# Bissmella/Small-object-detection-transformers

Hardware: AMD Instinct MI355X
Metric: images/sec (1024x1024 RGB+IR) train fwd+bwd (higher is better)
Workload: dtype bf16; 1 GPU; SRyolo_MF.yaml (model.yaml graph), batch 8/GPU @ 1024x1024 RGB+IR, fwd + hand-written bwd + fused SGD-nesterov/weight-decay + EMA step, loss = YOLOv5 ComputeLoss (CIoU + BCE, device kernels), 32 synthetic boxes/image, random-init weights; global_batch=8, parallelism=dp1

## Files before the change

### small-object-detection-transformers_amd/csrc/convmlp.hip

```cpp
#include "common.h"
#include "launch.h"
#include "../../include/sodt_hip.h"

namespace {

constexpr int CT = 64, CK = 16;
constexpr int CONVMLP_MAXC = 384;
template <typename LA, typename LB>
__device__ __forceinline__ void tile64(float (&acc)[4][4], int K, float (*As)[CT + 1], float (*Bs)[CT + 1], LA la, LB lb, bool a_k_fast, bool b_k_fast) {
  const int tid = threadIdx.x, ty = tid >> 4, tx = tid & 15;
  float pa[4], pb[4];
  auto fetch = [&](int k0) {
#pragma unroll
    for (int e = 0; e < 4; ++e) {
      const int idx = tid + 256 * e;
      pa[e] = a_k_fast ? la(idx >> 4, k0 + (idx & 15)) : la(idx & 63, k0 + (idx >> 6));
      pb[e] = b_k_fast ? lb(k0 + (idx & 15), idx >> 4) : lb(k0 + (idx >> 6), idx & 63);
    }
  };
  fetch(0);
  for (int k0 = 0; k0 < K; k0 += CK) {
#pragma unroll
    for (int e = 0; e < 4; ++e) {
      const int idx = tid + 256 * e;
      if (a_k_fast) As[idx & 15][idx >> 4] = pa[e]; else As[idx >> 6][idx & 63] = pa[e];
      if (b_k_fast) Bs[idx & 15][idx >> 4] = pb[e]; else Bs[idx >> 6][idx & 63] = pb[e];
    }
    __syncthreads();
    if (k0 + CK < K) fetch(k0 + CK);
#pragma unroll
    for (int k = 0; k < CK; ++k) {
      float a[4], b[4];
#pragma unroll
      for (int i = 0; i < 4; ++i) { a[i] = As[k][ty + 16 * i]; b[i] = Bs[k][tx + 16 * i]; }
#pragma unroll
      for (int i = 0; i < 4; ++i)
#pragma unroll
        for (int j = 0; j < 4; ++j) acc[i][j] = fmaf(a[i], b[j], acc[i][j]);
    }
    __syncthreads();
  }
}

__global__ __launch_bounds__(256) void convmlp_compose_kernel(const float* __restrict__ W1, const float* __restrict__ b1,
                                                              const float* __restrict__ Wc, const float* __restrict__ bc,
                                                              bf16* __restrict__ weff, bf16* __restrict__ weffT,
                                                              float* __restrict__ beff, float* __restrict__ vtap, int C) {
  __shared__ float As[CT][CT + 1], Bs[CK][CT + 1];
  const int tid = threadIdx.x, t = blockIdx.z;
  if ((int)blockIdx.y == C / CT) {
    if (t != 0 || (int)blockIdx.x * 32 >= C) return;
    const int co = blockIdx.x * 32 + (tid >> 3), part = tid & 7;
    float a[4] = {0.f, 0.f, 0.f, 0.f};
    for (int m = part; m < C; m += 8) {
      const float4 w = *(const float4*)(Wc + ((long)co * C + m) * 4);
      const float b = b1[m];
      a[0] = fmaf(w.x, b, a[0]); a[1] = fmaf(w.y, b, a[1]); a[2] = fmaf(w.z, b, a[2]); a[3] = fmaf(w.w, b, a[3]);
    }
#pragma unroll
    for (int j = 0; j < 4; ++j) { a[j] += __shfl_xor(a[j], 1); a[j] += __shfl_xor(a[j], 2); a[j] += __shfl_xor(a[j], 4); }
    if (part == 0) {
#pragma unroll
      for (int j = 0; j < 4; ++j) vtap[j * C + co] = a[j];
      beff[co] = bc[co] + a[0] + a[1] + a[2] + a[3];
    }
    return;
  }
  if ((int)blockIdx.x >= C / CT) return;
  const int ci0 = blockIdx.x * CT, co0 = blockIdx.y * CT;
  float acc[4][4] = {};
  tile64(acc, C, (float (*)[CT + 1])As, Bs,
         [&](int r, int k) { return Wc[((long)(co0 + r) * C + k) * 4 + t]; },
         [&](int k, int c) { return W1[(long)k * C + ci0 + c]; }, true, false);
  const int ty = tid >> 4, tx = tid & 15;
#pragma unroll
  for (int i = 0; i < 4; ++i)
#pragma unroll
    for (int j = 0; j < 4; ++j) {
      weff[(long)(co0 + ty + 16 * i) * 4 * C + t * C + ci0 + tx + 16 * j] = (bf16)acc[i][j];
      As[tx + 16 * j][ty + 16 * i] = acc[i][j];
    }
  __syncthreads();
  for (int idx = tid; idx < CT * CT; idx += 256) {
    const int r = idx >> 6, c = idx & 63;
    weffT[(long)(ci0 + r) * 4 * C + t * C + co0 + c] = (bf16)As[r][c];
  }
}

__global__ __launch_bounds__(256) void convmlp_border_fix_kernel(bf16* __restrict__ cp, bf16* __restrict__ ca, const float* __restrict__ vtap,
                                                                 int B, int H, int W, int C) {
  const int nb = H + W - 1, cpr = C / 8;
  const long i = (long)blockIdx.x * 256 + threadIdx.x;
  if (i >= (long)B * nb * cpr) return;
  const int c8 = (int)(i % cpr) * 8;
  const int k = (int)((i / cpr) % nb), b = (int)(i / ((long)cpr * nb));
  const int y = k < W ? H - 1 : k - W, x = k < W ? k : W - 1;
  const bool bot = y == H - 1, rgt = x == W - 1;
  const long row = ((long)b * H + y) * W + x;
  float v[8];
  unpack<bf16>(*(const uint4*)(cp + row * C + c8), v);
#pragma unroll
  for (int j = 0; j < 8; ++j) {
    float s = 0.f;
    if (rgt) s += vtap[1 * C + c8 + j];
    if (bot) s += vtap[2 * C + c8 + j];
    if (rgt || bot) s += vtap[3 * C + c8 + j];
    v[j] -= s;
  }
  *(uint4*)(cp + row * C + c8) = pack<bf16>(v);
#pragma unroll
  for (int j = 0; j < 8; ++j) v[j] = gelu_t<bf16>(v[j]);
  *(uint4*)(ca + row * C + c8) = pack<bf16>(v);
}

__global__ __launch_bounds__(256) void convmlp_border_sums_kernel(const bf16* __restrict__ dc, float* __restrict__ bs, int B, int H, int W, int C) {
  __shared__ float red[8][392];
  const int b = blockIdx.y, kind = blockIdx.z;
  const int len = kind == 0 ? H : W;
  const int t = blockIdx.x * 8 + (threadIdx.x >> 5);
  const int cpr = C / 8;
  const bool ok = t < len;
  const int y = kind == 0 ? t : H - 1, x = kind == 0 ? W - 1 : t;
  for (int ch = threadIdx.x & 31; ch < cpr; ch += 32) {
    float v[8] = {0.f, 0.f, 0.f, 0.f, 0.f, 0.f, 0.f, 0.f};
    if (ok) unpack<bf16>(*(const uint4*)(dc + (((long)b * H + y) * W + x) * C + ch * 8), v);
#pragma unroll
    for (int j = 0; j < 8; ++j) red[threadIdx.x >> 5][ch * 8 + j] = v[j];
    if (ok && kind == 0 && t == H - 1)
#pragma unroll
      for (int j = 0; j < 8; ++j) atomicAdd(bs + 2 * C + ch * 8 + j, v[j]);
  }
  __syncthreads();
  for (int c = threadIdx.x; c < C; c += 256) {
    float a = 0.f;
#pragma unroll
    for (int r = 0; r < 8; ++r) a += red[r][c];
    atomicAdd(bs + kind * C + c, a);
  }
}

__global__ __launch_bounds__(256) void convmlp_decompose_kernel(const float* __restrict__ dweff, const float* __restrict__ colsum,
                                                                const float* __restrict__ bs, const float* __restrict__ W1,
                                                                const float* __restrict__ b1, const float* __restrict__ Wc,
                                                                float* __restrict__ gWc, float* __restrict__ gbc, float* __restrict__ gW1,
                                                                float* __restrict__ gb1, int C) {
  __shared__ float As[CK][CT + 1], Bs[CK][CT + 1];
  __shared__ float dvs[4 * CONVMLP_MAXC];
  const int tid = threadIdx.x, ty = tid >> 4, tx = tid & 15;
  const int nt = C / CT, n = nt * nt;
  auto dv = [&](int t, int co) {
    const float r = bs[co], bt = bs[C + co], cn = bs[2 * C + co];
    return colsum[co] - (t == 0 ? 0.f : t == 1 ? r : t == 2 ? bt : r + bt - cn);
  };
  int bid = blockIdx.x;
  if (bid < 4 * n) {
    const int t = bid & 3, tl = bid >> 2;
    const int m0 = (tl % nt) * CT, co0 = (tl / nt) * CT;
    float acc[4][4] = {};
    tile64(acc, C, As, Bs,
           [&](int r, int k) { return dweff[(long)(co0 + r) * 4 * C + t * C + k]; },
           [&](int k, int c) { return W1[(long)(m0 + c) * C + k]; }, true, true);
#pragma unroll
    for (int i = 0; i < 4; ++i)
#pragma unroll
      for (int j = 0; j < 4; ++j)
        gWc[((long)(co0 + ty + 16 * i) * C + m0 + tx + 16 * j) * 4 + t] += acc[i][j] + dv(t, co0 + ty + 16 * i) * b1[m0 + tx + 16 * j];
    return;
  }
  bid -= 4 * n;
  if (bid < 4 * n) {
    const int q = bid & 3, tl = bid >> 2;
    const int ci0 = (tl % nt) * CT, m0 = (tl / nt) * CT;
    const int kq = q * C;
    float acc[4][4] = {};
    tile64(acc, C, As, Bs,
           [&](int r, int k) { const int kk = kq + k; return Wc[((long)(kk >> 2) * C + m0 + r) * 4 + (kk & 3)]; },
           [&](int k, int c) { const int kk = kq + k; return dweff[(long)(kk >> 2) * 4 * C + (kk & 3) * C + ci0 + c]; }, true, false);
#pragma unroll
    for (int i = 0; i < 4; ++i)
#pragma unroll
      for (int j = 0; j < 4; ++j) atomicAdd(gW1 + (long)(m0 + ty + 16 * i) * C + ci0 + tx + 16 * j, acc[i][j]);
    return;
  }
  bid -= 4 * n;
  for (int i = tid; i < 4 * C; i += 256) dvs[i] = dv(i / C, i % C);
  __syncthreads();
  const int m = bid * 32 + (tid >> 3), part = tid & 7;
  float acc = 0.f;
  for (int co = part; co < C; co += 8) {
    const float4 wc = *(const float4*)(Wc + ((long)co * C + m) * 4);
    acc += wc.x * dvs[co] + wc.y * dvs[C + co] + wc.z * dvs[2 * C + co] + wc.w * dvs[3 * C + co];
  }
  acc += __shfl_xor(acc, 1); acc += __shfl_xor(acc, 2); acc += __shfl_xor(acc, 4);
  if (part == 0) {
    gb1[m] += acc;
    gbc[m] += colsum[m];
  }
}

inline int nblk(long n) { return (int)((n + 255) / 256); }

}

extern "C" int sodt_convmlp_compose(const float* fc1_w, const float* fc1_b, const float* conv_w, const float* conv_b, void* weff,
                                    void* weffT, float* beff, float* vtap, int C, int dtype, sodt_stream_t st) {
  if (!fc1_w || !fc1_b || !conv_w || !conv_b || !weff || !weffT || !beff || !vtap || C <= 0 || (C % 64) || dtype != SODT_BF16 ||
      (((uintptr_t)conv_w) & 15))
    return SODT_EINVAL;
  return sodt_launch<convmlp_compose_kernel>(dim3(C / 32, C / 64 + 1, 4), dim3(256), 0, (hipStream_t)st, fc1_w, fc1_b, conv_w, conv_b,
                     (bf16*)weff, (bf16*)weffT, beff, vtap, C);
}

extern "C" int sodt_convmlp_border_fix(void* cp, void* ca, const float* vtap, int B, int H, int W, int C, int dtype, sodt_stream_t st) {
  if (!cp || !ca || !vtap || B <= 0 || H <= 0 || W <= 0 || C <= 0 || (C % 8) || dtype != SODT_BF16 ||
      ((((uintptr_t)cp) | ((uintptr_t)ca)) & 15))
    return SODT_EINVAL;
  return sodt_launch<convmlp_border_fix_kernel>(dim3(nblk((long)B * (H + W - 1) * (C / 8))), dim3(256), 0, (hipStream_t)st, (bf16*)cp,
                     (bf16*)ca, vtap, B, H, W, C);
}

extern "C" int sodt_convmlp_border_sums(const void* dc, float* bs, int B, int H, int W, int C, int dtype, sodt_stream_t st) {
  if (!dc || !bs || B <= 0 || H <= 0 || W <= 0 || C <= 0 || (C % 8) || C > 384 || dtype != SODT_BF16 || B > 65535 || (((uintptr_t)dc) & 15))
    return SODT_EINVAL;
  const int len = H > W ? H : W;
  return sodt_launch<convmlp_border_sums_kernel>(dim3((len + 7) / 8, B, 2), dim3(256), 0, (hipStream_t)st, (const bf16*)dc, bs, B, H, W, C);
}

extern "C" int sodt_convmlp_decompose(const float* dweff, const float* colsum, const float* bs, const float* fc1_w, const float* fc1_b,
                                      const float* conv_w, float* g_conv_w, float* g_conv_b, float* g_fc1_w, float* g_fc1_b, int C,
                                      sodt_stream_t st) {
  if (!dweff || !colsum || !bs || !fc1_w || !fc1_b || !conv_w || !g_conv_w || !g_conv_b || !g_fc1_w || !g_fc1_b || C <= 0 || (C % 64) ||
      C > CONVMLP_MAXC || ((((uintptr_t)conv_w) | ((uintptr_t)g_conv_w)) & 15))
    return SODT_EINVAL;
  const int n = (C / 64) * (C / 64);
  return sodt_launch<convmlp_decompose_kernel>(dim3(8 * n + C / 32), dim3(256), 0, (hipStream_t)st, dweff, colsum, bs, fc1_w, fc1_b, conv_w,
                     g_conv_w, g_conv_b, g_fc1_w, g_fc1_b, C);
}
```

### small-object-detection-transformers_amd/csrc/frontend.hip

```cpp
#include "common.h"
#include "launch.h"
#include "../../include/sodt_hip.h"

namespace {

constexpr int CE = 48;
constexpr int EP = CE + 1;
constexpr int FE_PART = 4 * CE * 19;
constexpr int FE_BWD_GRID = 512;

struct FeGeo { int B, H, W, th, tw; long ir_bstride; };

__device__ __forceinline__ void load_patch(const float* __restrict__ rgb, const float* __restrict__ ir, const FeGeo& g,
                                           int p, int b, int y, int x, float* pt) {
  const int H = g.H, W = g.W;
  const long plane = (long)H * W;
  if (p == 0) {
    const float* base = rgb + (long)b * 3 * plane;
#pragma unroll
    for (int i = 0; i < 4; ++i) {
      const int yy = 4 * y - 1 + i;
#pragma unroll
      for (int j = 0; j < 4; ++j) {
        const int xx = 4 * x - 1 + j;
        pt[i * 4 + j] = (yy >= 0 && xx >= 0 && yy < H && xx < W) ? base[(long)yy * W + xx] : 0.f;
      }
    }
  } else {
    const float* base = (p == 3) ? (ir + (long)b * g.ir_bstride) : (rgb + ((long)b * 3 + p) * plane);
#pragma unroll
    for (int i = 0; i < 4; ++i) {
      const float4 v = *(const float4*)(base + (long)(4 * y + i) * W + 4 * x);
      pt[i * 4] = v.x; pt[i * 4 + 1] = v.y; pt[i * 4 + 2] = v.z; pt[i * 4 + 3] = v.w;
    }
  }
}

__device__ __forceinline__ int pair_q(int q) { return q; }
__device__ __forceinline__ int pair_kv(int q) { return q == 0 ? 1 : (q == 1 ? 2 : (q == 2 ? 3 : 1)); }

template <typename T>
__global__ __launch_bounds__(256) void frontend_fwd_kernel(const float* __restrict__ rgb, const float* __restrict__ ir,
                                                          const float* __restrict__ w, const float* __restrict__ bias,
                                                          const float* __restrict__ gamma, const float* __restrict__ beta,
                                                          T* __restrict__ out, const FeGeo g, long ntok) {
  __shared__ float sE[4][64][EP];
  __shared__ __attribute__((aligned(16))) T sO[64 * 192];
  float (*sP)[64][17] = (float (*)[64][17])sO;
  static_assert(4 * 64 * 17 * 4 <= 64 * 192 * sizeof(T), "patch tile aliases the output tile");
  const int tid = threadIdx.x, lane = tid & 63;
  const int p = __builtin_amdgcn_readfirstlane(tid >> 6);
  const int t16 = lane & 15, g4 = lane >> 4;
  const long tok0 = (long)blockIdx.x * 64;
  const long tok = tok0 + lane;
  const bool live = tok < ntok;
  const int tt = g.th * g.tw;
  int b = 0, y = 0, x = 0;
  if (live) { b = (int)(tok / tt); const int rem = (int)(tok - (long)b * tt); y = rem / g.tw; x = rem - y * g.tw; }
  float pt[16];
  if (live) load_patch(rgb, ir, g, p, b, y, x, pt);
  else {
#pragma unroll
    for (int i = 0; i < 16; ++i) pt[i] = 0.f;
  }
  const float* wp = w + p * CE * 16;
  const float* bp = bias + p * CE;
#pragma unroll
  for (int k = 0; k < 16; ++k) sP[p][lane][k] = pt[k];
  wave_sync();
#pragma unroll
  for (int n = 0; n < 4; ++n) {
    float pb[4];
#pragma unroll
    for (int kk = 0; kk < 4; ++kk) pb[kk] = sP[p][16 * n + t16][4 * kk + g4];
#pragma unroll
    for (int s = 0; s < 3; ++s) {
      f32x4 e;
#pragma unroll
      for (int r = 0; r < 4; ++r) e[r] = bp[16 * s + 4 * g4 + r];
#pragma unroll
      for (int kk = 0; kk < 4; ++kk) e = __builtin_amdgcn_mfma_f32_16x16x4f32(wp[(16 * s + t16) * 16 + 4 * kk + g4], pb[kk], e, 0, 0, 0);
#pragma unroll
      for (int r = 0; r < 4; ++r) sE[p][16 * n + t16][16 * s + 4 * g4 + r] = e[r];
    }
  }
  __syncthreads();
  const int qa = pair_q(p), qb = pair_kv(p);
  float s[CE];
  float mean = 0.f;
#pragma unroll
  for (int j = 0; j < CE; ++j) { s[j] = sE[qa][lane][j] + sE[qb][lane][j]; mean += s[j]; }
  mean *= (1.0f / CE);
  float var = 0.f;
#pragma unroll
  for (int j = 0; j < CE; ++j) { const float d = s[j] - mean; var += d * d; }
  const float rstd = rsqrtf(var * (1.0f / CE) + 1e-5f);
  const float* gp = gamma + p * CE;
  const float* bt = beta + p * CE;
#pragma unroll
  for (int j = 0; j < CE; ++j) sO[lane * 192 + p * CE + j] = from_f<T>((s[j] - mean) * rstd * gp[j] + bt[j]);
  __syncthreads();
  constexpr int KPL = TT<T>::KPL;
  const long nvalid = (ntok - tok0) < 64 ? (ntok - tok0) : 64;
  for (int idx = tid; idx < 64 * 192 / KPL; idx += 256) {
    if ((long)idx * KPL < nvalid * 192) *(uint4*)(out + tok0 * 192 + (long)idx * KPL) = *(const uint4*)(sO + idx * KPL);
  }
}

template <typename T> __device__ __forceinline__ float chunk_elem(const uint4& u, int e);
template <> __device__ __forceinline__ float chunk_elem<float>(const uint4& u, int e) {
  return __uint_as_float(e == 0 ? u.x : (e == 1 ? u.y : (e == 2 ? u.z : u.w)));
}
template <> __device__ __forceinline__ float chunk_elem<bf16>(const uint4& u, int e) {
  const uint32_t wd = (e >> 1) == 0 ? u.x : ((e >> 1) == 1 ? u.y : ((e >> 1) == 2 ? u.z : u.w));
  return __uint_as_float((e & 1) ? (wd & 0xffff0000u) : (wd << 16));
}

__device__ __forceinline__ float fold4(const float* v) {
  auto a = __builtin_amdgcn_permlane32_swap(__float_as_uint(v[0]), __float_as_uint(v[2]), false, false);
  auto b = __builtin_amdgcn_permlane32_swap(__float_as_uint(v[1]), __float_as_uint(v[3]), false, false);
  const float sa = __uint_as_float(a[0]) + __uint_as_float(a[1]);
  const float sb = __uint_as_float(b[0]) + __uint_as_float(b[1]);
  auto c = __builtin_amdgcn_permlane16_swap(__float_as_uint(sa), __float_as_uint(sb), false, false);
  return __uint_as_float(c[0]) + __uint_as_float(c[1]);
}

template <int NQ>
__device__ __forceinline__ void dw_tiles(const float* d0, const float* d1, const float* d2, const float* pp, int lane,
                                         f32x4* adw) {
  const int t16 = lane & 15, g4 = lane >> 4;
#pragma unroll 4
  for (int kk = 0; kk < 16; ++kk) {
    const int tk = 4 * kk + g4;
    const float bv = pp[tk * 17 + t16];
#pragma unroll
    for (int s = 0; s < 3; ++s) {
      float av = d0[tk * EP + 16 * s + t16];
      if constexpr (NQ > 1) av += d1[tk * EP + 16 * s + t16];
      if constexpr (NQ > 2) av += d2[tk * EP + 16 * s + t16];
      adw[s] = __builtin_amdgcn_mfma_f32_16x16x4f32(av, bv, adw[s], 0, 0, 0);
    }
  }
}

template <typename T, bool WS>
__global__ __launch_bounds__(256, 2) void frontend_bwd_kernel(const float* __restrict__ rgb, const float* __restrict__ ir,
                                                             const float* __restrict__ w, const float* __restrict__ bias,
                                                             const float* __restrict__ gamma, const T* __restrict__ dout,
                                                             float* __restrict__ dw, float* __restrict__ db,
                                                             float* __restrict__ dgamma, float* __restrict__ dbeta,
                                                             float* __restrict__ ws, const FeGeo g, long ntok, int nblk) {
  __shared__ float sE[4][64][EP];
  __shared__ float sP[4][64][17];
  const int tid = threadIdx.x, lane = tid & 63;
  const int p = __builtin_amdgcn_readfirstlane(tid >> 6);
  const int tt = g.th * g.tw;
  const float* wp = w + p * CE * 16;
  const float* bp = bias + p * CE;
  const float* gp = gamma + p * CE;
  const int t16 = lane & 15, g4 = lane >> 4;
  constexpr int KPL = TT<T>::KPL, SPR = CE / KPL;

  f32x4 adw[3];
#pragma unroll
  for (int s = 0; s < 3; ++s) adw[s] = f32x4{0.f, 0.f, 0.f, 0.f};
  float adg[12], adbt[12], ads[12];
#pragma unroll
  for (int j = 0; j < 12; ++j) { adg[j] = 0.f; adbt[j] = 0.f; ads[j] = 0.f; }

  auto fetch = [&](int blk, float* pt) {
    const long tok = (long)blk * 64 + lane;
    if (blk < nblk && tok < ntok) {
      const int b = (int)(tok / tt);
      const int rem = (int)(tok - (long)b * tt);
      const int y = rem / g.tw, x = rem - y * g.tw;
      load_patch(rgb, ir, g, p, b, y, x, pt);
    } else {
#pragma unroll
      for (int i = 0; i < 16; ++i) pt[i] = 0.f;
    }
  };
  float pt[16];
  fetch(blockIdx.x, pt);
  float wa[3][4];
  f32x4 eb[3];
#pragma unroll
  for (int s = 0; s < 3; ++s) {
#pragma unroll
    for (int kk = 0; kk < 4; ++kk) wa[s][kk] = wp[(16 * s + t16) * 16 + 4 * kk + g4];
#pragma unroll
    for (int r = 0; r < 4; ++r) eb[s][r] = bp[16 * s + 4 * g4 + r];
  }

  for (int blk = blockIdx.x; blk < nblk; blk += gridDim.x) {
    const long tok = (long)blk * 64 + lane;
    const bool live = tok < ntok;
    uint4 raw[SPR];
#pragma unroll
    for (int c = 0; c < SPR; ++c)
      raw[c] = live ? *(const uint4*)(dout + tok * 192 + p * CE + c * KPL) : make_uint4(0u, 0u, 0u, 0u);
    __syncthreads();
#pragma unroll
    for (int k = 0; k < 16; ++k) sP[p][lane][k] = pt[k];
    wave_sync();
#pragma unroll
    for (int n = 0; n < 4; ++n) {
      float pb[4];
#pragma unroll
      for (int kk = 0; kk < 4; ++kk) pb[kk] = sP[p][16 * n + t16][4 * kk + g4];
#pragma unroll
      for (int s = 0; s < 3; ++s) {
        f32x4 e = eb[s];
#pragma unroll
        for (int kk = 0; kk < 4; ++kk) e = __builtin_amdgcn_mfma_f32_16x16x4f32(wa[s][kk], pb[kk], e, 0, 0, 0);
#pragma unroll
        for (int r = 0; r < 4; ++r) sE[p][16 * n + t16][16 * s + 4 * g4 + r] = e[r];
      }
    }
    __syncthreads();
    const int qa = pair_q(p), qb = pair_kv(p);
    float xh[CE];
    float mean = 0.f;
#pragma unroll
    for (int j0 = 0; j0 < CE; j0 += 12) {
#pragma unroll
      for (int j = j0; j < j0 + 12; ++j) { xh[j] = sE[qa][lane][j] + sE[qb][lane][j]; mean += xh[j]; }
      __builtin_amdgcn_sched_barrier(0);
    }
    __syncthreads();
    mean *= (1.0f / CE);
    float var = 0.f;
#pragma unroll
    for (int j = 0; j < CE; ++j) { xh[j] -= mean; var += xh[j] * xh[j]; }
    const float rstd = rsqrtf(var * (1.0f / CE) + 1e-5f);
    float c1 = 0.f, c2 = 0.f;
#pragma unroll
    for (int j = 0; j < 12; ++j) {
      float u[4], d[4];
#pragma unroll
      for (int m = 0; m < 4; ++m) {
        const int jj = j + 12 * m;
        d[m] = chunk_elem<T>(raw[jj / KPL], jj % KPL);
        xh[jj] *= rstd;
        const float gg = d[m] * gp[jj];
        c1 += gg; c2 += gg * xh[jj];
        u[m] = d[m] * xh[jj];
      }
      adg[j] += fold4(u);
      adbt[j] += fold4(d);
      __builtin_amdgcn_sched_barrier(0);
    }
    c1 *= (1.0f / CE); c2 *= (1.0f / CE);
#pragma unroll
    for (int j = 0; j < 12; ++j) {
      float d[4];
#pragma unroll
      for (int m = 0; m < 4; ++m) {
        const int jj = j + 12 * m;
        d[m] = rstd * (chunk_elem<T>(raw[jj / KPL], jj % KPL) * gp[jj] - c1 - xh[jj] * c2);
        sE[p][lane][jj] = d[m];
      }
      ads[j] += fold4(d);
    }
    fetch(blk + gridDim.x, pt);
    __syncthreads();
    if (p == 0) dw_tiles<1>(&sE[0][0][0], nullptr, nullptr, &sP[0][0][0], lane, adw);
    else if (p == 1) dw_tiles<3>(&sE[0][0][0], &sE[1][0][0], &sE[3][0][0], &sP[1][0][0], lane, adw);
    else if (p == 2) dw_tiles<2>(&sE[1][0][0], &sE[2][0][0], nullptr, &sP[2][0][0], lane, adw);
    else dw_tiles<2>(&sE[2][0][0], &sE[3][0][0], nullptr, &sP[3][0][0], lane, adw);
  }
  float* wsp = WS ? ws + (long)blockIdx.x * FE_PART + p * (FE_PART / 4) : nullptr;
#pragma unroll
  for (int s = 0; s < 3; ++s)
#pragma unroll
    for (int r = 0; r < 4; ++r) {
      const int o = (16 * s + 4 * g4 + r) * 16 + t16;
      if constexpr (WS) wsp[o] = adw[s][r];
      else atomicAdd(dw + p * CE * 16 + o, adw[s][r]);
    }
#pragma unroll
  for (int j = 0; j < 12; ++j) {
    float a = adg[j], c = adbt[j], d = ads[j];
#pragma unroll
    for (int m = 1; m < 16; m <<= 1) { a += __shfl_xor(a, m); c += __shfl_xor(c, m); d += __shfl_xor(d, m); }
    if (t16 == 0) {
      const int ch = j + 12 * g4;
      if constexpr (WS) {
        wsp[CE * 16 + ch] = a; wsp[CE * 17 + ch] = c; wsp[CE * 18 + ch] = d;
      } else {
        atomicAdd(dgamma + p * CE + ch, a);
        atomicAdd(dbeta + p * CE + ch, c);
        atomicAdd(db + pair_q(p) * CE + ch, d);
        atomicAdd(db + pair_kv(p) * CE + ch, d);
      }
    }
  }
}
// ... 1 lines not shown
constexpr int FE_RG = 32;
__global__ __launch_bounds__(64) void frontend_bwd_reduce_kernel(const float* __restrict__ ws, int nwg, float* __restrict__ dw,
                                                                float* __restrict__ db, float* __restrict__ dgamma,
                                                                float* __restrict__ dbeta) {
  const int col = blockIdx.x * 64 + threadIdx.x;
  const int r0 = blockIdx.y * FE_RG, r1 = (r0 + FE_RG) < nwg ? (r0 + FE_RG) : nwg;
  float a = 0.f;
  for (int r = r0; r < r1; ++r) a += ws[(long)r * FE_PART + col];
  const int p = col / (FE_PART / 4), o = col - p * (FE_PART / 4);
  if (o < CE * 16) atomicAdd(dw + p * CE * 16 + o, a);
  else if (o < CE * 17) atomicAdd(dgamma + p * CE + o - CE * 16, a);
  else if (o < CE * 18) atomicAdd(dbeta + p * CE + o - CE * 17, a);
  else {
    atomicAdd(db + pair_q(p) * CE + o - CE * 18, a);
    atomicAdd(db + pair_kv(p) * CE + o - CE * 18, a);
  }
}

bool fe_geo(FeGeo& g, int B, int H, int W, long ir_bstride) {
  if (B <= 0 || H <= 0 || W <= 0 || (H % 4) || (W % 4)) return false;
  g.B = B; g.H = H; g.W = W; g.th = H / 4; g.tw = W / 4; g.ir_bstride = ir_bstride;
  return true;
}

}

extern "C" int sodt_frontend_fwd_hw(const float* rgb, const float* ir, long ir_bstride, const float* w, const float* b,
                                    const float* gamma, const float* beta, void* out, int B, int H, int W, int ca_ws,
                                    int dtype, sodt_stream_t st) {
  FeGeo g;
  if (!rgb || !ir || !w || !b || !gamma || !beta || !out || !fe_geo(g, B, H, W, ir_bstride)) return SODT_EINVAL;
  if (ca_ws != 1) return SODT_EINVAL;
  const long ntok = (long)B * g.th * g.tw;
  const unsigned blocks = (unsigned)((ntok + 63) / 64);
  if (dtype == SODT_BF16)
    return sodt_launch<frontend_fwd_kernel<bf16>>(dim3(blocks), dim3(256), 0, (hipStream_t)st, rgb, ir, w, b, gamma, beta, (bf16*)out, g, ntok);
  if (dtype == SODT_F32)
    return sodt_launch<frontend_fwd_kernel<float>>(dim3(blocks), dim3(256), 0, (hipStream_t)st, rgb, ir, w, b, gamma, beta, (float*)out, g, ntok);
  return SODT_EINVAL;
}

extern "C" int sodt_frontend_fwd(const float* rgb, const float* ir, long ir_bstride, const float* w, const float* b,
                                 const float* gamma, const float* beta, void* out, int B, int S, int ca_ws,
                                 int dtype, sodt_stream_t st) {
  return sodt_frontend_fwd_hw(rgb, ir, ir_bstride, w, b, gamma, beta, out, B, S, S, ca_ws, dtype, st);
}

extern "C" long sodt_frontend_bwd_hw_workspace_bytes(int B, int H, int W) {
  (void)B; (void)H; (void)W;
  return (long)FE_BWD_GRID * FE_PART * (long)sizeof(float);
}

extern "C" long sodt_frontend_bwd_workspace_bytes(int B, int S) { return sodt_frontend_bwd_hw_workspace_bytes(B, S, S); }

extern "C" int sodt_frontend_bwd_hw(const float* rgb, const float* ir, long ir_bstride, const float* w, const float* b,
                                    const float* gamma, const float* beta, const void* dout,
                                    float* dw, float* db, float* dgamma, float* dbeta, int B, int H, int W, int ca_ws,
                                    float* ws, long ws_bytes, int dtype, sodt_stream_t st) {
  (void)beta;
  FeGeo g;
  if (!rgb || !ir || !w || !b || !gamma || !dout || !dw || !db || !dgamma || !dbeta || !fe_geo(g, B, H, W, ir_bstride)) return SODT_EINVAL;
  if (ca_ws != 1) return SODT_EINVAL;
  if (dtype != SODT_BF16 && dtype != SODT_F32) return SODT_EINVAL;
  const long ntok = (long)B * g.th * g.tw;
  const int nblk = (int)((ntok + 63) / 64);
  const bool two_stage = ws && ws_bytes >= sodt_frontend_bwd_hw_workspace_bytes(B, H, W) && nblk > 64;
  const int cap = two_stage ? FE_BWD_GRID : FE_BWD_GRID / 2;
  const unsigned blocks = (unsigned)(nblk < cap ? nblk : cap);
  hipStream_t s = (hipStream_t)st;
#define FE_BWD_LAUNCH(T_, WS_) sodt_launch<frontend_bwd_kernel<T_, WS_>>(dim3(blocks), dim3(256), 0, s, rgb, ir, w, b, gamma, \
                                                  (const T_*)dout, dw, db, dgamma, dbeta, ws, g, ntok, nblk)
// ... 15 lines not shown
```

Measured before the change: 219.9 images/sec.

## Retile convmlp weight algebra kernels and make frontend forward persistent with prefetch

Replaces the generic 64x64 tile GEMM helper in the convmlp compose/decompose kernels with TM-templated panel GEMMs that stage vectorized float4 panels in LDS, fold the four conv taps into one block, and widen the K chunk. The bias-tail reductions are unrolled with batched loads. Separately, the frontend forward kernel becomes a grid-capped persistent loop that prefetches the next patch while computing, aliases its output tile onto the embedding LDS, and writes packed stores. This aims to cut launch/tail overhead and global load latency, at the cost of more registers and extra synchronization.

Measured after the change: 221.2 images/sec, median of 6. No clear change (+0.6%).

```diff
diff --git a/small-object-detection-transformers_amd/csrc/convmlp.hip b/small-object-detection-transformers_amd/csrc/convmlp.hip
--- a/small-object-detection-transformers_amd/csrc/convmlp.hip
+++ b/small-object-detection-transformers_amd/csrc/convmlp.hip
@@ -4,58 +4,69 @@
 
 namespace {
 
-constexpr int CT = 64, CK = 16;
+constexpr int AKC = 192;
+constexpr int ALG_LDS = 16000;
 constexpr int CONVMLP_MAXC = 384;
-template <typename LA, typename LB>
-__device__ __forceinline__ void tile64(float (&acc)[4][4], int K, float (*As)[CT + 1], float (*Bs)[CT + 1], LA la, LB lb, bool a_k_fast, bool b_k_fast) {
-  const int tid = threadIdx.x, ty = tid >> 4, tx = tid & 15;
-  float pa[4], pb[4];
-  auto fetch = [&](int k0) {
-#pragma unroll
-    for (int e = 0; e < 4; ++e) {
-      const int idx = tid + 256 * e;
-      pa[e] = a_k_fast ? la(idx >> 4, k0 + (idx & 15)) : la(idx & 63, k0 + (idx >> 6));
-      pb[e] = b_k_fast ? lb(k0 + (idx & 15), idx >> 4) : lb(k0 + (idx >> 6), idx & 63);
-    }
-  };
-  fetch(0);
-  for (int k0 = 0; k0 < K; k0 += CK) {
-#pragma unroll
-    for (int e = 0; e < 4; ++e) {
-      const int idx = tid + 256 * e;
-      if (a_k_fast) As[idx & 15][idx >> 4] = pa[e]; else As[idx >> 6][idx & 63] = pa[e];
-      if (b_k_fast) Bs[idx & 15][idx >> 4] = pb[e]; else Bs[idx >> 6][idx & 63] = pb[e];
-    }
-    __syncthreads();
-    if (k0 + CK < K) fetch(k0 + CK);
-#pragma unroll
-    for (int k = 0; k < CK; ++k) {
-      float a[4], b[4];
-#pragma unroll
-      for (int i = 0; i < 4; ++i) { a[i] = As[k][ty + 16 * i]; b[i] = Bs[k][tx + 16 * i]; }
-#pragma unroll
-      for (int i = 0; i < 4; ++i)
-#pragma unroll
-        for (int j = 0; j < 4; ++j) acc[i][j] = fmaf(a[i], b[j], acc[i][j]);
-    }
-    __syncthreads();
-  }
-}
-
+constexpr int TAILB = 24;
+
+template <int IT4>
+__device__ __forceinline__ void panel_load(float4 (&v)[IT4], bool al, const float* __restrict__ src, long sld, int rows, int len, int tid) {
+  const int l4 = len >> 2, n = rows * l4;
+#pragma unroll
+  for (int it = 0; it < IT4; ++it) {
+    const int i = (tid + 256 * it) < n ? (tid + 256 * it) : (n - 1), r = i / l4, c = i - r * l4;
+    v[it] = al ? *(const float4*)(src + (long)r * sld + 4 * c) : make_float4(0.f, 0.f, 0.f, 0.f);
+  }
+}
+template <int IT4>
+__device__ __forceinline__ void panel_store(const float4 (&v)[IT4], bool al, float* dst, int dld, const float* __restrict__ src, long sld,
+                                            int rows, int len, int tid) {
+  if (al) {
+    const int l4 = len >> 2, n = rows * l4;
+#pragma unroll
+    for (int it = 0; it < IT4; ++it) {
+      const int i = tid + 256 * it, r = i / l4, c = i - r * l4;
+      if (i < n) *(float4*)(dst + r * dld + 4 * c) = v[it];
+    }
+  } else {
+    const int n = rows * len;
+#pragma unroll 8
+    for (int i = tid; i < n; i += 256) {
+      const int r = i / len, c = i - r * len;
+      dst[r * dld + c] = src[(long)r * sld + c];
+    }
+  }
+}
+__device__ __forceinline__ bool aligned16(const float* p, long ld) { return ((((uintptr_t)p) & 15) == 0) && ((ld & 3) == 0); }
+
+template <int TM>
 __global__ __launch_bounds__(256) void convmlp_compose_kernel(const float* __restrict__ W1, const float* __restrict__ b1,
                                                               const float* __restrict__ Wc, const float* __restrict__ bc,
                                                               bf16* __restrict__ weff, bf16* __restrict__ weffT,
                                                               float* __restrict__ beff, float* __restrict__ vtap, int C) {
-  __shared__ float As[CT][CT + 1], Bs[CK][CT + 1];
-  const int tid = threadIdx.x, t = blockIdx.z;
-  if ((int)blockIdx.y == C / CT) {
-    if (t != 0 || (int)blockIdx.x * 32 >= C) return;
-    const int co = blockIdx.x * 32 + (tid >> 3), part = tid & 7;
+  __shared__ __attribute__((aligned(16))) float smem[ALG_LDS];
+  constexpr int TW = 16 * TM, KC = AKC / TM;
+  const int tid = threadIdx.x;
+  const int nt = C / TW;
+  int bid = blockIdx.x;
+  if (bid >= nt * nt) {
+    bid -= nt * nt;
+    const int co = bid * 32 + (tid >> 3), part = tid & 7;
     float a[4] = {0.f, 0.f, 0.f, 0.f};
-    for (int m = part; m < C; m += 8) {
-      const float4 w = *(const float4*)(Wc + ((long)co * C + m) * 4);
-      const float b = b1[m];
-      a[0] = fmaf(w.x, b, a[0]); a[1] = fmaf(w.y, b, a[1]); a[2] = fmaf(w.z, b, a[2]); a[3] = fmaf(w.w, b, a[3]);
+    for (int mb = part; mb < C; mb += 8 * TAILB) {
+      float4 w[TAILB];
+      float b[TAILB];
+#pragma unroll
+      for (int u = 0; u < TAILB; ++u) {
+        const int m = (mb + 8 * u) < C ? (mb + 8 * u) : part;
+        w[u] = *(const float4*)(Wc + ((long)co * C + m) * 4);
+        b[u] = b1[m];
+      }
+#pragma unroll
+      for (int u = 0; u < TAILB; ++u)
+        if (mb + 8 * u < C) {
+          a[0] = fmaf(w[u].x, b[u], a[0]); a[1] = fmaf(w[u].y, b[u], a[1]); a[2] = fmaf(w[u].z, b[u], a[2]); a[3] = fmaf(w[u].w, b[u], a[3]);
+        }
     }
 #pragma unroll
     for (int j = 0; j < 4; ++j) { a[j] += __shfl_xor(a[j], 1); a[j] += __shfl_xor(a[j], 2); a[j] += __shfl_xor(a[j], 4); }
@@ -66,25 +77,69 @@
     }
     return;
   }
-  if ((int)blockIdx.x >= C / CT) return;
-  const int ci0 = blockIdx.x * CT, co0 = blockIdx.y * CT;
-  float acc[4][4] = {};
-  tile64(acc, C, (float (*)[CT + 1])As, Bs,
-         [&](int r, int k) { return Wc[((long)(co0 + r) * C + k) * 4 + t]; },
-         [&](int k, int c) { return W1[(long)k * C + ci0 + c]; }, true, false);
-  const int ty = tid >> 4, tx = tid & 15;
-#pragma unroll
-  for (int i = 0; i < 4; ++i)
-#pragma unroll
-    for (int j = 0; j < 4; ++j) {
-      weff[(long)(co0 + ty + 16 * i) * 4 * C + t * C + ci0 + tx + 16 * j] = (bf16)acc[i][j];
-      As[tx + 16 * j][ty + 16 * i] = acc[i][j];
-    }
+  const int co0 = (bid / nt) * TW, ci0 = (bid % nt) * TW;
+  const int r = tid >> 4, c = tid & 15;
+  constexpr int ARW = 4 * KC + 4;
+  float* sA = smem;
+  float* sB = smem + TW * ARW;
+  static_assert(TW * ARW + KC * TW <= ALG_LDS && 4 * TW * (TW + 1) <= ALG_LDS, "compose panels fit");
+  constexpr int ITA = TW * KC / 256, ITB = KC * TW / 1024;
+  const bool alA = aligned16(Wc, 4), alB = aligned16(W1, C);
+  float4 va[ITA], vb[ITB];
+  float acc[TM][TM][4] = {};
+  int kc = C < KC ? C : KC;
+  panel_load(va, alA, Wc + (long)co0 * C * 4, 4L * C, TW, 4 * kc, tid);
+  panel_load(vb, alB, W1 + ci0, C, kc, TW, tid);
+  for (int k0 = 0; k0 < C; k0 += KC) {
+    if (k0) __syncthreads();
+    panel_store(va, alA, sA, ARW, Wc + ((long)co0 * C + k0) * 4, 4L * C, TW, 4 * kc, tid);
+    panel_store(vb, alB, sB, TW, W1 + (long)k0 * C + ci0, C, kc, TW, tid);
+    __syncthreads();
+    const int kcur = kc;
+    if (k0 + KC < C) {
+      kc = (C - k0 - KC) < KC ? (C - k0 - KC) : KC;
+      panel_load(va, alA, Wc + ((long)co0 * C + k0 + KC) * 4, 4L * C, TW, 4 * kc, tid);
+      panel_load(vb, alB, W1 + (long)(k0 + KC) * C + ci0, C, kc, TW, tid);
+    }
+#pragma unroll 4
+    for (int m = 0; m < kcur; ++m) {
+      float4 a[TM];
+      float b[TM];
+#pragma unroll
+      for (int i = 0; i < TM; ++i) a[i] = *(const float4*)(sA + (r + 16 * i) * ARW + 4 * m);
+#pragma unroll
+      for (int j = 0; j < TM; ++j) b[j] = sB[m * TW + c + 16 * j];
+#pragma unroll
+      for (int i = 0; i < TM; ++i)
+#pragma unroll
+        for (int j = 0; j < TM; ++j) {
+          acc[i][j][0] = fmaf(a[i].x, b[j], acc[i][j][0]); acc[i][j][1] = fmaf(a[i].y, b[j], acc[i][j][1]);
+          acc[i][j][2] = fmaf(a[i].z, b[j], acc[i][j][2]); acc[i][j][3] = fmaf(a[i].w, b[j], acc[i][j][3]);
+        }
+    }
+  }
+#pragma unroll
+  for (int i = 0; i < TM; ++i)
+#pragma unroll
+    for (int j = 0; j < TM; ++j)
+#pragma unroll
+      for (int t = 0; t < 4; ++t) weff[(long)(co0 + r + 16 * i) * 4 * C + t * C + ci0 + c + 16 * j] = (bf16)acc[i][j][t];
   __syncthreads();
-  for (int idx = tid; idx < CT * CT; idx += 256) {
-    const int r = idx >> 6, c = idx & 63;
-    weffT[(long)(ci0 + r) * 4 * C + t * C + co0 + c] = (bf16)As[r][c];
-  }
+  float* sT = smem;
+#pragma unroll
+  for (int i = 0; i < TM; ++i)
+#pragma unroll
+    for (int j = 0; j < TM; ++j)
+#pragma unroll
+      for (int t = 0; t < 4; ++t) sT[(t * TW + c + 16 * j) * (TW + 1) + r + 16 * i] = acc[i][j][t];
+  __syncthreads();
+#pragma unroll
+  for (int i = 0; i < TM; ++i)
+#pragma unroll
+    for (int j = 0; j < TM; ++j)
+#pragma unroll
+      for (int t = 0; t < 4; ++t)
+        weffT[(long)(ci0 + r + 16 * i) * 4 * C + t * C + co0 + c + 16 * j] = (bf16)sT[(t * TW + r + 16 * i) * (TW + 1) + c + 16 * j];
 }
 
 __global__ __launch_bounds__(256) void convmlp_border_fix_kernel(bf16* __restrict__ cp, bf16* __restrict__ ca, const float* __restrict__ vtap,
@@ -139,57 +194,145 @@
   }
 }
 
+__host__ __device__ inline int decompose_kq(int C, int TM) { return ((C % 192) == 0 ? 96 : 64) / TM; }
+__host__ __device__ inline int algebra_tm(int C) { return C > 192 ? 2 : 1; }
+
+template <int TM>
 __global__ __launch_bounds__(256) void convmlp_decompose_kernel(const float* __restrict__ dweff, const float* __restrict__ colsum,
                                                                 const float* __restrict__ bs, const float* __restrict__ W1,
                                                                 const float* __restrict__ b1, const float* __restrict__ Wc,
                                                                 float* __restrict__ gWc, float* __restrict__ gbc, float* __restrict__ gW1,
                                                                 float* __restrict__ gb1, int C) {
-  __shared__ float As[CK][CT + 1], Bs[CK][CT + 1];
-  __shared__ float dvs[4 * CONVMLP_MAXC];
-  const int tid = threadIdx.x, ty = tid >> 4, tx = tid & 15;
-  const int nt = C / CT, n = nt * nt;
+  __shared__ __attribute__((aligned(16))) float smem[ALG_LDS];
+  static_assert(4 * CONVMLP_MAXC <= ALG_LDS, "dv[t][co] of the bias tail fits");
+  constexpr int TW = 16 * TM, KC = AKC / TM, ALD = KC + 4;
+  const int tid = threadIdx.x, r = tid >> 4, c = tid & 15;
+  const int nt = C / TW, n = nt * nt;
   auto dv = [&](int t, int co) {
-    const float r = bs[co], bt = bs[C + co], cn = bs[2 * C + co];
-    return colsum[co] - (t == 0 ? 0.f : t == 1 ? r : t == 2 ? bt : r + bt - cn);
+    const float rr = bs[co], bt = bs[C + co], cn = bs[2 * C + co];
+    return colsum[co] - (t == 0 ? 0.f : t == 1 ? rr : t == 2 ? bt : rr + bt - cn);
   };
   int bid = blockIdx.x;
-  if (bid < 4 * n) {
-    const int t = bid & 3, tl = bid >> 2;
-    const int m0 = (tl % nt) * CT, co0 = (tl / nt) * CT;
-    float acc[4][4] = {};
-    tile64(acc, C, As, Bs,
-           [&](int r, int k) { return dweff[(long)(co0 + r) * 4 * C + t * C + k]; },
-           [&](int k, int c) { return W1[(long)(m0 + c) * C + k]; }, true, true);
-#pragma unroll
-    for (int i = 0; i < 4; ++i)
-#pragma unroll
-      for (int j = 0; j < 4; ++j)
-        gWc[((long)(co0 + ty + 16 * i) * C + m0 + tx + 16 * j) * 4 + t] += acc[i][j] + dv(t, co0 + ty + 16 * i) * b1[m0 + tx + 16 * j];
+  if (bid < n) {
+    const int m0 = (bid % nt) * TW, co0 = (bid / nt) * TW;
+    float* sA = smem;
+    float* sB = smem + 4 * TW * ALD;
+    static_assert(5 * TW * ALD <= ALG_LDS, "conv1.weight panels fit");
+    constexpr int ITA = 4 * TW * KC / 1024, ITB = TW * KC / 1024;
+    const bool alA = aligned16(dweff, C), alB = aligned16(W1, C);
+    float4 va[ITA], vb[ITB];
+    float acc[TM][TM][4] = {};
+    int kc = C < KC ? C : KC;
+    panel_load(va, alA, dweff + (long)co0 * 4 * C, C, 4 * TW, kc, tid);
+    panel_load(vb, alB, W1 + (long)m0 * C, C, TW, kc, tid);
+    for (int k0 = 0; k0 < C; k0 += KC) {
+      if (k0) __syncthreads();
+      panel_store(va, alA, sA, ALD, dweff + (long)co0 * 4 * C + k0, C, 4 * TW, kc, tid);
+      panel_store(vb, alB, sB, ALD, W1 + (long)m0 * C + k0, C, TW, kc, tid);
+      __syncthreads();
+      const int kcur = kc;
+      if (k0 + KC < C) {
+        kc = (C - k0 - KC) < KC ? (C - k0 - KC) : KC;
+        panel_load(va, alA, dweff + (long)co0 * 4 * C + k0 + KC, C, 4 * TW, kc, tid);
+        panel_load(vb, alB, W1 + (long)m0 * C + k0 + KC, C, TW, kc, tid);
+      }
+#pragma unroll 2
+      for (int k = 0; k < kcur; k += 4) {
+        float4 b[TM];
+#pragma unroll
+        for (int j = 0; j < TM; ++j) b[j] = *(const float4*)(sB + (c + 16 * j) * ALD + k);
+#pragma unroll
+        for (int i = 0; i < TM; ++i)
+#pragma unroll
+          for (int t = 0; t < 4; ++t) {
+            const float4 a = *(const float4*)(sA + (4 * (r + 16 * i) + t) * ALD + k);
+#pragma unroll
+            for (int j = 0; j < TM; ++j) {
+              float v = acc[i][j][t];
+              v = fmaf(a.x, b[j].x, v); v = fmaf(a.y, b[j].y, v); v = fmaf(a.z, b[j].z, v); v = fmaf(a.w, b[j].w, v);
+              acc[i][j][t] = v;
+            }
+          }
+      }
+    }
+#pragma unroll
+    for (int i = 0; i < TM; ++i)
+#pragma unroll
+      for (int j = 0; j < TM; ++j) {
+        const int co = co0 + r + 16 * i, m = m0 + c + 16 * j;
+        float4* gp = (float4*)(gWc + ((long)co * C + m) * 4);
+        const float bm = b1[m];
+        float4 g = *gp;
+        g.x += acc[i][j][0] + dv(0, co) * bm; g.y += acc[i][j][1] + dv(1, co) * bm;
+        g.z += acc[i][j][2] + dv(2, co) * bm; g.w += acc[i][j][3] + dv(3, co) * bm;
+        *gp = g;
+      }
     return;
   }
-  bid -= 4 * n;
-  if (bid < 4 * n) {
-    const int q = bid & 3, tl = bid >> 2;
-    const int ci0 = (tl % nt) * CT, m0 = (tl / nt) * CT;
-    const int kq = q * C;
-    float acc[4][4] = {};
-    tile64(acc, C, As, Bs,
-           [&](int r, int k) { const int kk = kq + k; return Wc[((long)(kk >> 2) * C + m0 + r) * 4 + (kk & 3)]; },
-           [&](int k, int c) { const int kk = kq + k; return dweff[(long)(kk >> 2) * 4 * C + (kk & 3) * C + ci0 + c]; }, true, false);
-#pragma unroll
-    for (int i = 0; i < 4; ++i)
-#pragma unroll
-      for (int j = 0; j < 4; ++j) atomicAdd(gW1 + (long)(m0 + ty + 16 * i) * C + ci0 + tx + 16 * j, acc[i][j]);
+  bid -= n;
+  const int kq = decompose_kq(C, TM), nq = C / kq;
+  if (bid < n * nq) {
+    const int q = bid % nq, tl = bid / nq;
+    const int ci0 = (tl % nt) * TW, m0 = (tl / nt) * TW, cq = q * kq;
+    constexpr int KQ = 96 / TM;
+    float* sA = smem;
+    float* sB = smem + KQ * 4 * TW;
+    static_assert(2 * KQ * 4 * TW <= ALG_LDS, "fc1.weight panels fit");
+    constexpr int IT = KQ * TW / 256;
+    const bool alA = aligned16(Wc, 4), alB = aligned16(dweff, C);
+    float4 va[IT], vb[IT];
+    panel_load(va, alA, Wc + ((long)cq * C + m0) * 4, 4L * C, kq, 4 * TW, tid);
+    panel_load(vb, alB, dweff + (long)cq * 4 * C + ci0, C, 4 * kq, TW, tid);
+    panel_store(va, alA, sA, 4 * TW, Wc + ((long)cq * C + m0) * 4, 4L * C, kq, 4 * TW, tid);
+    panel_store(vb, alB, sB, TW, dweff + (long)cq * 4 * C + ci0, C, 4 * kq, TW, tid);
+    __syncthreads();
+    float acc[TM][TM] = {};
+#pragma unroll 4
+    for (int j = 0; j < kq; ++j) {
+      float4 a[TM];
+      float b[4][TM];
+#pragma unroll
+      for (int i = 0; i < TM; ++i) a[i] = *(const float4*)(sA + (j * TW + r + 16 * i) * 4);
+#pragma unroll
+      for (int t = 0; t < 4; ++t)
+#pragma unroll
+        for (int jj = 0; jj < TM; ++jj) b[t][jj] = sB[(4 * j + t) * TW + c + 16 * jj];
+#pragma unroll
+      for (int i = 0; i < TM; ++i)
+#pragma unroll
+        for (int jj = 0; jj < TM; ++jj) {
+          float v = acc[i][jj];
+          v = fmaf(a[i].x, b[0][jj], v); v = fmaf(a[i].y, b[1][jj], v); v = fmaf(a[i].z, b[2][jj], v); v = fmaf(a[i].w, b[3][jj], v);
+          acc[i][jj] = v;
+        }
+    }
+#pragma unroll
+    for (int i = 0; i < TM; ++i)
+#pragma unroll
+      for (int jj = 0; jj < TM; ++jj) atomicAdd(gW1 + (long)(m0 + r + 16 * i) * C + ci0 + c + 16 * jj, acc[i][jj]);
     return;
   }
-  bid -= 4 * n;
-  for (int i = tid; i < 4 * C; i += 256) dvs[i] = dv(i / C, i % C);
+  bid -= n * nq;
+  float* dvs = smem;
+  for (int co = tid; co < C; co += 256) {
+#pragma unroll
+    for (int t = 0; t < 4; ++t) dvs[t * C + co] = dv(t, co);
+  }
   __syncthreads();
   const int m = bid * 32 + (tid >> 3), part = tid & 7;
   float acc = 0.f;
-  for (int co = part; co < C; co += 8) {
-    const float4 wc = *(const float4*)(Wc + ((long)co * C + m) * 4);
-    acc += wc.x * dvs[co] + wc.y * dvs[C + co] + wc.z * dvs[2 * C + co] + wc.w * dvs[3 * C + co];
+  for (int cb = part; cb < C; cb += 8 * TAILB) {
+    float4 w[TAILB];
+#pragma unroll
+    for (int u = 0; u < TAILB; ++u) {
+      const int co = (cb + 8 * u) < C ? (cb + 8 * u) : part;
+      w[u] = *(const float4*)(Wc + ((long)co * C + m) * 4);
+    }
+#pragma unroll
+    for (int u = 0; u < TAILB; ++u) {
+      const int co = cb + 8 * u;
+      if (co < C) acc += w[u].x * dvs[co] + w[u].y * dvs[C + co] + w[u].z * dvs[2 * C + co] + w[u].w * dvs[3 * C + co];
+    }
   }
   acc += __shfl_xor(acc, 1); acc += __shfl_xor(acc, 2); acc += __shfl_xor(acc, 4);
   if (part == 0) {
@@ -207,8 +350,13 @@
   if (!fc1_w || !fc1_b || !conv_w || !conv_b || !weff || !weffT || !beff || !vtap || C <= 0 || (C % 64) || dtype != SODT_BF16 ||
       (((uintptr_t)conv_w) & 15))
     return SODT_EINVAL;
-  return sodt_launch<convmlp_compose_kernel>(dim3(C / 32, C / 64 + 1, 4), dim3(256), 0, (hipStream_t)st, fc1_w, fc1_b, conv_w, conv_b,
-                     (bf16*)weff, (bf16*)weffT, beff, vtap, C);
+  const int tm = algebra_tm(C), nt = C / (16 * tm);
+  const dim3 grid(nt * nt + C / 32);
+  if (tm == 1)
+    return sodt_launch<convmlp_compose_kernel<1>>(grid, dim3(256), 0, (hipStream_t)st, fc1_w, fc1_b, conv_w, conv_b, (bf16*)weff,
+                       (bf16*)weffT, beff, vtap, C);
+  return sodt_launch<convmlp_compose_kernel<2>>(grid, dim3(256), 0, (hipStream_t)st, fc1_w, fc1_b, conv_w, conv_b, (bf16*)weff,
+                     (bf16*)weffT, beff, vtap, C);
 }
 
 extern "C" int sodt_convmlp_border_fix(void* cp, void* ca, const float* vtap, int B, int H, int W, int C, int dtype, sodt_stream_t st) {
@@ -232,7 +380,11 @@
   if (!dweff || !colsum || !bs || !fc1_w || !fc1_b || !conv_w || !g_conv_w || !g_conv_b || !g_fc1_w || !g_fc1_b || C <= 0 || (C % 64) ||
       C > CONVMLP_MAXC || ((((uintptr_t)conv_w) | ((uintptr_t)g_conv_w)) & 15))
     return SODT_EINVAL;
-  const int n = (C / 64) * (C / 64);
-  return sodt_launch<convmlp_decompose_kernel>(dim3(8 * n + C / 32), dim3(256), 0, (hipStream_t)st, dweff, colsum, bs, fc1_w, fc1_b, conv_w,
-                     g_conv_w, g_conv_b, g_fc1_w, g_fc1_b, C);
-}
+  const int tm = algebra_tm(C), n = (C / (16 * tm)) * (C / (16 * tm));
+  const dim3 grid(n + n * (C / decompose_kq(C, tm)) + C / 32);
+  if (tm == 1)
+    return sodt_launch<convmlp_decompose_kernel<1>>(grid, dim3(256), 0, (hipStream_t)st, dweff, colsum, bs, fc1_w, fc1_b, conv_w, g_conv_w,
+                       g_conv_b, g_fc1_w, g_fc1_b, C);
+  return sodt_launch<convmlp_decompose_kernel<2>>(grid, dim3(256), 0, (hipStream_t)st, dweff, colsum, bs, fc1_w, fc1_b, conv_w, g_conv_w,
+                     g_conv_b, g_fc1_w, g_fc1_b, C);
+}
diff --git a/small-object-detection-transformers_amd/csrc/frontend.hip b/small-object-detection-transformers_amd/csrc/frontend.hip
--- a/small-object-detection-transformers_amd/csrc/frontend.hip
+++ b/small-object-detection-transformers_amd/csrc/frontend.hip
@@ -8,30 +8,52 @@
 constexpr int EP = CE + 1;
 constexpr int FE_PART = 4 * CE * 19;
 constexpr int FE_BWD_GRID = 512;
+constexpr int FE_FWD_GRID = 768;
 
 struct FeGeo { int B, H, W, th, tw; long ir_bstride; };
 
+struct PatchRaw { float4 v[4]; float e[4]; int left; };
+
+__device__ __forceinline__ void patch_zero(PatchRaw& r) {
+#pragma unroll
+  for (int i = 0; i < 4; ++i) { r.v[i] = make_float4(0.f, 0.f, 0.f, 0.f); r.e[i] = 0.f; }
+  r.left = 0;
+}
+
 __device__ __forceinline__ void load_patch(const float* __restrict__ rgb, const float* __restrict__ ir, const FeGeo& g,
-                                           int p, int b, int y, int x, float* pt) {
-  const int H = g.H, W = g.W;
-  const long plane = (long)H * W;
+                                           int p, int b, int y, int x, int lane, PatchRaw& r) {
+  const int W = g.W;
+  const long plane = (long)g.H * W;
   if (p == 0) {
     const float* base = rgb + (long)b * 3 * plane;
+    r.left = x == 0 ? 0 : (lane == 0 ? 2 : 1);
 #pragma unroll
     for (int i = 0; i < 4; ++i) {
       const int yy = 4 * y - 1 + i;
-#pragma unroll
-      for (int j = 0; j < 4; ++j) {
-        const int xx = 4 * x - 1 + j;
-        pt[i * 4 + j] = (yy >= 0 && xx >= 0 && yy < H && xx < W) ? base[(long)yy * W + xx] : 0.f;
-      }
+      const float* row = base + (long)yy * W + 4 * x;
+      r.v[i] = yy >= 0 ? *(const float4*)row : make_float4(0.f, 0.f, 0.f, 0.f);
+      r.e[i] = (yy >= 0 && r.left == 2) ? row[-1] : 0.f;
     }
   } else {
     const float* base = (p == 3) ? (ir + (long)b * g.ir_bstride) : (rgb + ((long)b * 3 + p) * plane);
+    r.left = 0;
 #pragma unroll
     for (int i = 0; i < 4; ++i) {
-      const float4 v = *(const float4*)(base + (long)(4 * y + i) * W + 4 * x);
-      pt[i * 4] = v.x; pt[i * 4 + 1] = v.y; pt[i * 4 + 2] = v.z; pt[i * 4 + 3] = v.w;
+      r.v[i] = *(const float4*)(base + (long)(4 * y + i) * W + 4 * x);
+      r.e[i] = 0.f;
+    }
+  }
+}
+
+__device__ __forceinline__ void patch_taps(int p, const PatchRaw& r, float* pt) {
+#pragma unroll
+  for (int i = 0; i < 4; ++i) {
+    if (p == 0) {
+      const float nb = __shfl_up(r.v[i].w, 1);
+      pt[i * 4] = r.left == 1 ? nb : r.e[i];
+      pt[i * 4 + 1] = r.v[i].x; pt[i * 4 + 2] = r.v[i].y; pt[i * 4 + 3] = r.v[i].z;
+    } else {
+      pt[i * 4] = r.v[i].x; pt[i * 4 + 1] = r.v[i].y; pt[i * 4 + 2] = r.v[i].z; pt[i * 4 + 3] = r.v[i].w;
     }
   }
 }
@@ -40,70 +62,103 @@
 __device__ __forceinline__ int pair_kv(int q) { return q == 0 ? 1 : (q == 1 ? 2 : (q == 2 ? 3 : 1)); }
 
 template <typename T>
-__global__ __launch_bounds__(256) void frontend_fwd_kernel(const float* __restrict__ rgb, const float* __restrict__ ir,
+__global__ __launch_bounds__(256, 3) void frontend_fwd_kernel(const float* __restrict__ rgb, const float* __restrict__ ir,
                                                           const float* __restrict__ w, const float* __restrict__ bias,
                                                           const float* __restrict__ gamma, const float* __restrict__ beta,
-                                                          T* __restrict__ out, const FeGeo g, long ntok) {
-  __shared__ float sE[4][64][EP];
-  __shared__ __attribute__((aligned(16))) T sO[64 * 192];
-  float (*sP)[64][17] = (float (*)[64][17])sO;
-  static_assert(4 * 64 * 17 * 4 <= 64 * 192 * sizeof(T), "patch tile aliases the output tile");
+                                                          T* __restrict__ out, const FeGeo g, long ntok, int nblk) {
+  constexpr int KPL = TT<T>::KPL, CPR = 192 / KPL;
+  constexpr int RS = 192 * (int)sizeof(T) + 16;
+  __shared__ __attribute__((aligned(16))) float sE[4][64][EP];
+  static_assert(64 * RS <= (int)sizeof(float) * 4 * 64 * EP, "the output tile aliases the embeddings");
+  static_assert(64 * 17 <= 64 * EP, "a wave's patch tile fits its plane's slot");
+  unsigned char* sO = (unsigned char*)&sE[0][0][0];
   const int tid = threadIdx.x, lane = tid & 63;
   const int p = __builtin_amdgcn_readfirstlane(tid >> 6);
+  float (*sP)[17] = (float (*)[17])&sE[p][0][0];
   const int t16 = lane & 15, g4 = lane >> 4;
-  const long tok0 = (long)blockIdx.x * 64;
-  const long tok = tok0 + lane;
-  const bool live = tok < ntok;
   const int tt = g.th * g.tw;
-  int b = 0, y = 0, x = 0;
-  if (live) { b = (int)(tok / tt); const int rem = (int)(tok - (long)b * tt); y = rem / g.tw; x = rem - y * g.tw; }
-  float pt[16];
-  if (live) load_patch(rgb, ir, g, p, b, y, x, pt);
-  else {
-#pragma unroll
-    for (int i = 0; i < 16; ++i) pt[i] = 0.f;
-  }
   const float* wp = w + p * CE * 16;
   const float* bp = bias + p * CE;
-#pragma unroll
-  for (int k = 0; k < 16; ++k) sP[p][lane][k] = pt[k];
-  wave_sync();
-#pragma unroll
-  for (int n = 0; n < 4; ++n) {
-    float pb[4];
-#pragma unroll
-    for (int kk = 0; kk < 4; ++kk) pb[kk] = sP[p][16 * n + t16][4 * kk + g4];
-#pragma unroll
-    for (int s = 0; s < 3; ++s) {
-      f32x4 e;
-#pragma unroll
-      for (int r = 0; r < 4; ++r) e[r] = bp[16 * s + 4 * g4 + r];
-#pragma unroll
-      for (int kk = 0; kk < 4; ++kk) e = __builtin_amdgcn_mfma_f32_16x16x4f32(wp[(16 * s + t16) * 16 + 4 * kk + g4], pb[kk], e, 0, 0, 0);
-#pragma unroll
-      for (int r = 0; r < 4; ++r) sE[p][16 * n + t16][16 * s + 4 * g4 + r] = e[r];
-    }
-  }
-  __syncthreads();
-  const int qa = pair_q(p), qb = pair_kv(p);
-  float s[CE];
-  float mean = 0.f;
-#pragma unroll
-  for (int j = 0; j < CE; ++j) { s[j] = sE[qa][lane][j] + sE[qb][lane][j]; mean += s[j]; }
-  mean *= (1.0f / CE);
-  float var = 0.f;
-#pragma unroll
-  for (int j = 0; j < CE; ++j) { const float d = s[j] - mean; var += d * d; }
-  const float rstd = rsqrtf(var * (1.0f / CE) + 1e-5f);
   const float* gp = gamma + p * CE;
   const float* bt = beta + p * CE;
-#pragma unroll
-  for (int j = 0; j < CE; ++j) sO[lane * 192 + p * CE + j] = from_f<T>((s[j] - mean) * rstd * gp[j] + bt[j]);
-  __syncthreads();
-  constexpr int KPL = TT<T>::KPL;
-  const long nvalid = (ntok - tok0) < 64 ? (ntok - tok0) : 64;
-  for (int idx = tid; idx < 64 * 192 / KPL; idx += 256) {
-    if ((long)idx * KPL < nvalid * 192) *(uint4*)(out + tok0 * 192 + (long)idx * KPL) = *(const uint4*)(sO + idx * KPL);
+  const int qa = pair_q(p), qb = pair_kv(p);
+
+  auto fetch = [&](int blk, PatchRaw& r) {
+    const long tok = (long)blk * 64 + lane;
+    if (blk < nblk && tok < ntok) {
+      const int b = (int)(tok / tt);
+      const int rem = (int)(tok - (long)b * tt);
+      const int y = rem / g.tw, x = rem - y * g.tw;
+      load_patch(rgb, ir, g, p, b, y, x, lane, r);
+    } else {
+      patch_zero(r);
+    }
+  };
+  PatchRaw raw;
+  fetch(blockIdx.x, raw);
+  float wa[3][4];
+  f32x4 eb[3];
+#pragma unroll
+  for (int s = 0; s < 3; ++s) {
+#pragma unroll
+    for (int kk = 0; kk < 4; ++kk) wa[s][kk] = wp[(16 * s + t16) * 16 + 4 * kk + g4];
+#pragma unroll
+    for (int r = 0; r < 4; ++r) eb[s][r] = bp[16 * s + 4 * g4 + r];
+  }
+
+  for (int blk = blockIdx.x; blk < nblk; blk += gridDim.x) {
+    const long tok0 = (long)blk * 64;
+    float pt[16];
+    patch_taps(p, raw, pt);
+    __syncthreads();
+#pragma unroll
+    for (int k = 0; k < 16; ++k) sP[lane][k] = pt[k];
+    wave_sync();
+    float pb[4][4];
+#pragma unroll
+    for (int n = 0; n < 4; ++n)
+#pragma unroll
+      for (int kk = 0; kk < 4; ++kk) pb[n][kk] = sP[16 * n + t16][4 * kk + g4];
+    wave_sync();
+    fetch(blk + gridDim.x, raw);
+#pragma unroll
+    for (int n = 0; n < 4; ++n) {
+#pragma unroll
+      for (int s = 0; s < 3; ++s) {
+        f32x4 e = eb[s];
+#pragma unroll
+        for (int kk = 0; kk < 4; ++kk) e = __builtin_amdgcn_mfma_f32_16x16x4f32(wa[s][kk], pb[n][kk], e, 0, 0, 0);
+#pragma unroll
+        for (int r = 0; r < 4; ++r) sE[p][16 * n + t16][16 * s + 4 * g4 + r] = e[r];
+      }
+    }
+    __syncthreads();
+    float s[CE];
+    float mean = 0.f;
+#pragma unroll
+    for (int j = 0; j < CE; ++j) { s[j] = sE[qa][lane][j] + sE[qb][lane][j]; mean += s[j]; }
+    __syncthreads();
+    mean *= (1.0f / CE);
+    float var = 0.f;
+#pragma unroll
+    for (int j = 0; j < CE; ++j) { const float d = s[j] - mean; var += d * d; }
+    const float rstd = rsqrtf(var * (1.0f / CE) + 1e-5f);
+#pragma unroll
+    for (int c = 0; c < CE / KPL; ++c) {
+      float o[KPL];
+#pragma unroll
+      for (int e = 0; e < KPL; ++e) {
+        const int j = c * KPL + e;
+        o[e] = (s[j] - mean) * rstd * gp[j] + bt[j];
+      }
+      *(uint4*)(sO + lane * RS + (p * CE + c * KPL) * (int)sizeof(T)) = pack<T>(o);
+    }
+    __syncthreads();
+    const long nvalid = (ntok - tok0) < 64 ? (ntok - tok0) : 64;
+    for (int idx = tid; idx < 64 * CPR; idx += 256) {
+      const int row = idx / CPR, c = idx - row * CPR;
+      if (row < nvalid) *(uint4*)(out + (tok0 + row) * 192 + c * KPL) = *(const uint4*)(sO + row * RS + c * 16);
+    }
   }
 }
 
@@ -168,20 +223,19 @@
 #pragma unroll
   for (int j = 0; j < 12; ++j) { adg[j] = 0.f; adbt[j] = 0.f; ads[j] = 0.f; }
 
-  auto fetch = [&](int blk, float* pt) {
+  auto fetch = [&](int blk, PatchRaw& r) {
     const long tok = (long)blk * 64 + lane;
     if (blk < nblk && tok < ntok) {
       const int b = (int)(tok / tt);
       const int rem = (int)(tok - (long)b * tt);
       const int y = rem / g.tw, x = rem - y * g.tw;
-      load_patch(rgb, ir, g, p, b, y, x, pt);
+      load_patch(rgb, ir, g, p, b, y, x, lane, r);
     } else {
-#pragma unroll
-      for (int i = 0; i < 16; ++i) pt[i] = 0.f;
+      patch_zero(r);
     }
   };
-  float pt[16];
-  fetch(blockIdx.x, pt);
+  PatchRaw pr;
+  fetch(blockIdx.x, pr);
   float wa[3][4];
   f32x4 eb[3];
 #pragma unroll
@@ -199,6 +253,8 @@
 #pragma unroll
     for (int c = 0; c < SPR; ++c)
       raw[c] = live ? *(const uint4*)(dout + tok * 192 + p * CE + c * KPL) : make_uint4(0u, 0u, 0u, 0u);
+    float pt[16];
+    patch_taps(p, pr, pt);
     __syncthreads();
 #pragma unroll
     for (int k = 0; k < 16; ++k) sP[p][lane][k] = pt[k];
@@ -262,7 +318,7 @@
       }
       ads[j] += fold4(d);
     }
-    fetch(blk + gridDim.x, pt);
+    fetch(blk + gridDim.x, pr);
     __syncthreads();
     if (p == 0) dw_tiles<1>(&sE[0][0][0], nullptr, nullptr, &sP[0][0][0], lane, adw);
     else if (p == 1) dw_tiles<3>(&sE[0][0][0], &sE[1][0][0], &sE[3][0][0], &sP[1][0][0], lane, adw);
@@ -330,11 +386,12 @@
   if (!rgb || !ir || !w || !b || !gamma || !beta || !out || !fe_geo(g, B, H, W, ir_bstride)) return SODT_EINVAL;
   if (ca_ws != 1) return SODT_EINVAL;
   const long ntok = (long)B * g.th * g.tw;
-  const unsigned blocks = (unsigned)((ntok + 63) / 64);
+  const int nblk = (int)((ntok + 63) / 64);
+  const unsigned blocks = (unsigned)(nblk < FE_FWD_GRID ? nblk : FE_FWD_GRID);
   if (dtype == SODT_BF16)
-    return sodt_launch<frontend_fwd_kernel<bf16>>(dim3(blocks), dim3(256), 0, (hipStream_t)st, rgb, ir, w, b, gamma, beta, (bf16*)out, g, ntok);
+    return sodt_launch<frontend_fwd_kernel<bf16>>(dim3(blocks), dim3(256), 0, (hipStream_t)st, rgb, ir, w, b, gamma, beta, (bf16*)out, g, ntok, nblk);
   if (dtype == SODT_F32)
-    return sodt_launch<frontend_fwd_kernel<float>>(dim3(blocks), dim3(256), 0, (hipStream_t)st, rgb, ir, w, b, gamma, beta, (float*)out, g, ntok);
+    return sodt_launch<frontend_fwd_kernel<float>>(dim3(blocks), dim3(256), 0, (hipStream_t)st, rgb, ir, w, b, gamma, beta, (float*)out, g, ntok, nblk);
   return SODT_EINVAL;
 }
 
```
